# genome/breakdancer

Hardware: AMD Instinct MI355X
Metric: read-pairs/s, records resident in HBM -> scored SV table (SURVEY 8d timing i); end to end from BAM: config.timings.bam_to_table (vs_baseline is taken there) (higher is better)
Workload: dtype int32

## Files before the change

breakdancer_amd/csrc/bdx_api.hip:

```cpp
#include <hip/hip_runtime.h>

#include <algorithm>
#include <atomic>
#include <functional>
#include <memory>
#include <chrono>
#include <cmath>
#include <cstdio>
#include <cstddef>
#include <cstring>
#include <string>
#include <thread>
#include <unordered_map>
#include <utility>
#include <vector>

#include "../../include/bdx.h"
#include "bdx_buf.h"
#include "bdx_dev.h"
#include "bdx_k3.h"
#include "bdx_shard.h"
#include "bdx_scan.h"
#include "bdx_walk.h"
#include "bdx_bam_dev.h"

using namespace bdx;

namespace {

struct KdScratch {
    DevBuf bits, longbits, cnt;
    DevBuf work, wrun, starts, pre, cbase, table, multi;
    void release_long() { work.release(); wrun.release(); starts.release(); pre.release(); cbase.release(); table.release(); multi.release(); }
};

struct StageBufs {
    DevBuf b_c_tid, b_c_pos, b_c_isize, b_c_meta, b_c_key, b_c_check, b_c_idx, b_c_nn, b_c_pk;
    DevBuf b_cand, b_pre_q, b_pre_rev, b_pre_nonctx, b_c_first, b_c_maxq, b_c_rid, b_region_of, b_lb;
    DevBuf b_bcnt, b_boff, b_bcur, b_e_key, b_e_idx, b_partner, b_t_key, b_t_idx, b_pair_lo;
    DevBuf b_groups;
    DevBuf b_r_rec, b_r_pk, b_out_deg, b_parts, b_rs, b_slot, b_members, b_own, b_lib_stage, b_cn_stage, b_t_lambda, b_t_k, b_ws6;
    DevBuf b_sv_src, b_dlists, b_ltail, b_ins, b_member_ids;
    DevBuf b_sv_out, b_lib_index_out, b_lib_pairs_out, b_cn_key_out, b_cn_value_out, b_ltail_out, b_sv_key;
    PinBuf h_regs, h_pk, h_groups, h_counts0, h_counts2, h_sv_out, h_lib_index, h_lib_pairs, h_cn_key, h_cn_value, h_ltail_dev;
};

constexpr int kNumStages = 12;
enum StageMs { kMsClassify, kMsCompact, kMsCut, kMsJoinAssemble, kMsGroupsWait, kMsHostWalk, kMsFinish, kMsRun, kMsTableWait, kMsMerge, kMsScores };
enum ReadyWord { kPass1Ready, kGroupsReady, kTableReady, kRegionsReady };
constexpr int kK1MaxGrid = 8192;
constexpr uint32_t kK1EventPeriod = 4;

}

struct bdx_ctx {
    int device = 0;
    Stream stream;
    Stream copy_stream;
    bdx_opts opts{};
    std::vector<bdx_lib> libs;
    int nlibs = 0, nbams = 0, ntids = 0, nkeys = 0, w0 = 0;
    std::string err;

    ReadsSoA d{};
    size_t n = 0, cap = 0;
    bool adopted = false;
    DevBuf b_tid, b_pos, b_mtid, b_mpos, b_isize, b_flag, b_qlen, b_mapq, b_lib, b_bam, b_key, b_check;
    bool groups_in_hbm = false;
    bool use_check = false;

    DevBuf b_libs, b_cls, b_tile_tot, b_tile_pre, b_tile_mono, b_blk_cnt, b_cnt, b_p1, b_fold, b_stash, b_chunk_tot, b_counts;
    DevBuf b_lib_mean, b_kdens;
    PinBuf h_p1, h_cnt, h_counts, h_terms;
    PinBuf h_hs_rec, h_hs_aux, h_hs_lists, h_printed;
    StageBufs sb;
    PinBuf h_flags;
    PinBuf h_count;
    uint32_t seq = 0;
    int dbg_no_stash = 0, dbg_max_chunks = 0, dbg_ins_plain = 0, dbg_gather_walk = 0, dbg_regions_copy = 0, dbg_asm_plain = 0, dbg_depth_plain = 0;
    uint32_t lb_seq = 0;
    float k1_ms_last = 0;
    bool k1_timed = false;
    bool stage_timing = false;
    bool poll = true;
    bool materialized = true;
    bool rows_packed = false;
    uint32_t n_sv_total = 0, n_groups_total = 0, n_terms_total = 0, n_cn_total = 0;
    Event ev_groups, ev_regions;
    int big_walk_mode = -1;
    int64_t last_big_groups = -1;
    FinalizeParams fp_deferred{};
    bool finalize2_deferred = false;
    bool bucketed_join = false;
    bool host_walk_only = false;
    K6Arrays k6{};
    const GroupRec* k6_in_groups = nullptr;
    const uint32_t* k6_in_goff = nullptr;
    bool force_direct_join = false;
    uint32_t k6_cap = 0;
    const RegionRec* k6_r_rec = nullptr;
    const uint32_t* k6_r_pk = nullptr;
    uint8_t* k6_taint = nullptr;
    bool table_in_hbm = false;

    bool ran = false;
    Pass1 p1{};
    StageCounts counts{};
    std::vector<uint32_t> cnt;
    std::vector<uint32_t> cnt_local;
    uint32_t g_covered = 0;
    int32_t g_window = 0;
    uint32_t ntiles = 0, tstride = 0;
    Compact cp{};
    K3Arrays k3{};
    K4Arrays k4{};
    std::vector<double> log_tail;
    bool collect_support = false;
    std::vector<uint32_t> ov_cnt;
    uint32_t ov_covered = 0;
    bool replayed = false;
    bool use_stash = false;
    std::atomic<int> sizing{0};
    std::string sizing_err;
    std::vector<uint32_t> sup_off;
    std::vector<uint64_t> sup_idx;
    std::vector<uint8_t> sup_flag;
    std::vector<float> seqcov, lib_density, key_density;
    std::vector<HostRegion> regions;
    std::vector<uint32_t> r_pk;
    const HostRegion* reg = nullptr;
    size_t nreg = 0;
    const uint32_t* rpk = nullptr;
    std::vector<GroupPart> parts;
    WalkResult walk;
    std::unique_ptr<WalkScratch, void (*)(WalkScratch*)> walk_scratch{nullptr, walk_scratch_free};
    uint32_t n_printed = 0;
    uint32_t n_sv_host = 0;
    int speculate = 2;
    int spec_test = 0;
    uint32_t last_na = 0;
    size_t last_n = 0;
    uint32_t count_chunks = 0;
    uint32_t na_alloc = 0;
    bool region_of_fused = false;
    uint32_t join_table_clean = 0;
    float stage_ms[kNumStages] = {0};
    Event ev[8];

    Event ev_copy;
    bool copy_pending = false;
    bool k1_live = false;
    uint32_t k1_done = 0, k1_cap_tiles = 0;
    struct Stage {
        PinBuf buf;
        size_t cap = 0;
        Event done;
        bool busy = false;
    };
    Stage ring[4];
    int ring_next = 0, ring_cur = -1;
    struct KeySeg { uint64_t begin; const uint64_t* host; const uint16_t* host_qlen; const uint64_t* host_check; };
    std::vector<KeySeg> key_segs;
    DevBuf b_seg;

    size_t cls_n = (size_t)-1;
    DevBuf b_qtab;
    DevBuf b_qin, b_qout;
    bool mark_dup = false;
    bool dup_done = false;
    uint64_t dup_marked = 0, dup_groups = 0;
    KdScratch kd;
};

namespace {

// ... 452 lines not shown

int kd_run(bdx_ctx* c, KdParams p, KdScratch& k, uint16_t* flag, uint8_t* mask, hipStream_t s, uint64_t* marked, uint64_t* groups) {
    if (!p.n) return BDX_OK;
    const size_t nwords = (p.n + 63) / 64;
    HIPCHK(c, k.bits.ensure(nwords * 8));
    HIPCHK(c, k.longbits.ensure(nwords * 8));
    HIPCHK(c, k.cnt.ensure(sizeof(KdCounts)));
    p.bits = k.bits.as<uint64_t>(); p.longbits = k.longbits.as<uint64_t>(); p.cnt = k.cnt.as<KdCounts>();
    HIPCHK(c, hipMemsetAsync(p.cnt, 0, sizeof(KdCounts), s));
    launch_kd_scan(p, s);
    HIPCHK(c, hipGetLastError());
    KdCounts h{};
    HIPCHK(c, hipMemcpyAsync(&h, p.cnt, sizeof(h), hipMemcpyDeviceToHost, s));
    HIPCHK(c, hipStreamSynchronize(s));
    if (h.nwork) {
        if (h.nwork > (1u << 30)) return fail(c, BDX_ELIMIT, "more than 2^30 duplicate candidates in runs too long for direct comparison");
        uint64_t slots = 1024;
        while (slots < 2 * (uint64_t)h.nwork) slots <<= 1;
        HIPCHK(c, k.work.ensure((size_t)h.nwork * 4));
        HIPCHK(c, k.wrun.ensure((size_t)h.nwork * 4));
        HIPCHK(c, k.starts.ensure(nwords * 8));
        HIPCHK(c, k.pre.ensure(nwords * 4));
        HIPCHK(c, k.cbase.ensure((size_t)kd_chunks(p.n) * 4));
        HIPCHK(c, k.table.ensure(slots * 4));
        HIPCHK(c, k.multi.ensure(slots * 4));
        p.work = k.work.as<uint32_t>(); p.wrun = k.wrun.as<uint32_t>(); p.starts = k.starts.as<uint64_t>();
        p.pre = k.pre.as<uint32_t>(); p.cbase = k.cbase.as<uint32_t>();
        p.table = k.table.as<uint32_t>(); p.multi = k.multi.as<uint32_t>(); p.tmask = slots - 1;
        launch_kd_long(p, h.nwork, s);
        HIPCHK(c, hipGetLastError());
    }
    launch_kd_apply(p, flag, mask, s);
    HIPCHK(c, hipGetLastError());
    if (h.nwork) {
        HIPCHK(c, hipMemcpyAsync(&h, p.cnt, sizeof(h), hipMemcpyDeviceToHost, s));
        HIPCHK(c, hipStreamSynchronize(s));
        if (h.nlist != h.nwork) return fail(c, BDX_EINTERNAL, "duplicate marking: the work list does not hold the candidates that were counted");
        k.release_long();
    }
    *marked += h.marked; *groups += h.groups;
    return BDX_OK;
}

int mark_duplicates(bdx_ctx* c) {
    if (c->dup_done) return BDX_OK;
    c->dup_marked = 0; c->dup_groups = 0;
    hipStream_t s = c->stream;
    if (c->adopted && (const void*)c->d.flag != c->b_flag.p) {
        HIPCHK(c, c->b_flag.ensure(c->n * 2));
        HIPCHK(c, hipMemcpyAsync(c->b_flag.p, c->d.flag, c->n * 2, hipMemcpyDeviceToDevice, s));
        c->d.flag = c->b_flag.as<uint16_t>();
    }
    KdParams p{};
    p.tid = c->d.tid; p.pos = c->d.pos; p.mtid = c->d.mtid; p.mpos = c->d.mpos; p.flag = c->d.flag;
    p.lib = c->nlibs > 1 ? c->d.lib : nullptr;
    p.key = c->d.key; p.n = c->n;
    size_t ns = 0;
    BDX_TRY(upload_key_segs(c, &ns));
    if (ns) {
        p.nseg = (int)ns;
        p.seg_begin = c->b_seg.as<uint64_t>();
        p.seg_ptr = (const uint64_t* const*)(c->b_seg.as<uint64_t>() + ns + 1);
    }
    BDX_TRY(kd_run(c, p, c->kd, (uint16_t*)c->d.flag, nullptr, s, &c->dup_marked, &c->dup_groups));
    c->dup_done = true;
    return BDX_OK;
}

int pass1_prepare(bdx_ctx* c, uint32_t tiles_cap) {
    HIPCHK(c, hipSetDevice(c->device));
    hipStream_t s = c->stream;
    const int nlibs = c->nlibs, nbams = c->nbams, nkeys = c->nkeys;
    const int ncols = 2 + nkeys, ncnt = nlibs * kNumFlags + nlibs + nbams;
    const uint32_t tstride = (uint32_t)round_up(std::max<uint32_t>(tiles_cap, 16), 16);
    c->tstride = tstride;
    c->k1_cap_tiles = tiles_cap;
    c->k1_done = 0;
    HIPCHK(c, c->b_cls.ensure(std::max<size_t>((size_t)tiles_cap * kTile, 16)));
    c->use_stash = !c->dbg_no_stash && nkeys <= kStashKeys;
    if (c->use_stash) HIPCHK(c, c->b_stash.ensure(std::max<size_t>((size_t)tiles_cap * kStashCap * sizeof(StashRec), 64)));
    HIPCHK(c, c->b_tile_tot.ensure((size_t)ncols * tstride * 4));
    HIPCHK(c, c->b_tile_pre.ensure((size_t)ncols * tstride * 4));
    HIPCHK(c, c->b_tile_mono.ensure((size_t)nbams * tstride * sizeof(MonoRec)));
    HIPCHK(c, c->b_blk_cnt.ensure((size_t)kCntCopies * ncnt * 4));
    HIPCHK(c, c->b_cnt.ensure((size_t)ncnt * 4));
    HIPCHK(c, c->b_p1.ensure(sizeof(Pass1)));
    HIPCHK(c, c->h_p1.ensure(sizeof(Pass1)));
    HIPCHK(c, c->h_cnt.ensure((size_t)ncnt * 4));
    HIPCHK(c, c->h_counts.ensure(sizeof(StageCounts)));
    HIPCHK(c, c->b_counts.ensure(sizeof(StageCounts)));
    HIPCHK(c, c->h_count.ensure((size_t)kMaxChunks * 8));
    const size_t w_tot = (size_t)ncols * tstride, w_mono = (size_t)nbams * tstride * sizeof(MonoRec) / 4;
    if (w_tot > 0xFFFFFFFFull || w_mono > 0xFFFFFFFFull) {
        HIPCHK(c, hipMemsetAsync(c->b_tile_tot.p, 0, w_tot * 4, s));
        HIPCHK(c, hipMemsetAsync(c->b_tile_mono.p, 0xFF, w_mono * 4, s));
    }
    InitList il{};
    int k = 0;
    auto add = [&](void* p, size_t words, uint32_t value) { il.ptr[k] = (uint32_t*)p; il.words[k] = (uint32_t)words; il.value[k] = value; ++k; };
    if (w_tot <= 0xFFFFFFFFull && w_mono <= 0xFFFFFFFFull) { add(c->b_tile_tot.p, w_tot, 0u); add(c->b_tile_mono.p, w_mono, 0xFFFFFFFFu); }
    add(c->b_blk_cnt.p, (size_t)kCntCopies * ncnt, 0u);
    add(c->b_p1.p, sizeof(Pass1) / 4, 0u);
    add(c->b_counts.p, sizeof(StageCounts) / 4, 0u);
    il.n = k;
    launch_init(il, s);
    return BDX_OK;
}

int pass1_classify(bdx_ctx* c, uint32_t upto, bool timed) {
    hipStream_t s = c->stream;
    if (upto <= c->k1_done) return BDX_OK;
    K1Params k1{};
    k1.r = c->d; k1.n = c->n; k1.ntiles = upto; k1.tstride = c->tstride; k1.tile0 = c->k1_done;
    k1.nlibs = c->nlibs; k1.nbams = c->nbams; k1.nkeys = c->nkeys;
    k1.max_sd = c->opts.max_sd; k1.opt_t = c->opts.transchr_rearrange; k1.opt_l = c->opts.illumina_long_insert;
    k1.libs = c->b_libs.as<DevLib>(); k1.cls = c->b_cls.as<uint8_t>(); k1.tile_tot = c->b_tile_tot.as<uint32_t>();
    k1.tile_mono = c->b_tile_mono.as<MonoRec>();
    k1.blk_cnt = c->b_blk_cnt.as<uint32_t>();
    k1.stash = c->use_stash ? c->b_stash.as<StashRec>() : nullptr;
    const uint32_t span = upto - c->k1_done;
    const int grid1 = (int)std::min<uint32_t>((span + kWaves - 1) / kWaves, (uint32_t)kK1MaxGrid);
    launch_k1(k1, grid1, k1_lds_bytes(c->nlibs, c->nbams, c->nkeys), s, timed ? c->ev[0] : nullptr, timed ? c->ev[1] : nullptr);
    c->k1_done = upto;
    return BDX_OK;
}

struct Pass1Launch {
    uint32_t na_cap = 0;
    bool defer_second = false;
    bool post_count = false;
};
int pass1_finalize(bdx_ctx* c, const Pass1Launch& opt) {
    const int nlibs = c->nlibs, nbams = c->nbams, nkeys = c->nkeys;
    const int ncols = 2 + nkeys, ncnt = nlibs * kNumFlags + nlibs + nbams;
    const uint32_t ntiles = c->ntiles;
    FinalizeParams fp{};
    fp.ntiles = ntiles; fp.tstride = c->tstride; fp.nblk = 0;
    fp.nfold = std::max<uint32_t>(1, std::min<uint32_t>(64, (ntiles + 1023) / 1024));
    HIPCHK(c, c->b_fold.ensure((size_t)nbams * fp.nfold * sizeof(MonoRec)));
    fp.fold_part = c->b_fold.as<MonoRec>();
    fp.nlibs = nlibs; fp.nbams = nbams; fp.nkeys = nkeys; fp.ncols = ncols; fp.ncnt = ncnt; fp.w0 = c->w0;
    fp.tile_tot = c->b_tile_tot.as<uint32_t>(); fp.tile_pre = c->b_tile_pre.as<uint32_t>(); fp.tile_mono = c->b_tile_mono.as<MonoRec>();
    {
        const uint32_t nsuper = (ntiles + kK2TilesPerWave - 1) / kK2TilesPerWave;
        const uint32_t round = 4096;
        const uint32_t rounds = std::max<uint32_t>(1, (nsuper + round - 1) / round);
        const uint32_t max_chunks = c->dbg_max_chunks > 0 ? (uint32_t)std::min(c->dbg_max_chunks, (int)kMaxChunks) : (uint32_t)kMaxChunks;
        fp.chunk_super = round * ((rounds + max_chunks - 1) / max_chunks);
        fp.nchunk = std::max<uint32_t>(1, (nsuper + fp.chunk_super - 1) / fp.chunk_super);
        HIPCHK(c, c->b_chunk_tot.ensure((size_t)ncols * kMaxChunks * 8));
        fp.chunk_tot = c->b_chunk_tot.as<uint32_t>();
        fp.chunk_base = fp.chunk_tot + (size_t)ncols * kMaxChunks;
    }
    fp.blk_cnt = c->b_blk_cnt.as<uint32_t>(); fp.cnt = c->b_cnt.as<uint32_t>(); fp.p1 = c->b_p1.as<Pass1>();
    HIPCHK(c, c->b_kdens.ensure(64 * 4));
    fp.libs = c->b_libs.as<DevLib>(); fp.cn_lib = c->opts.cn_lib; fp.key_density = c->b_kdens.as<float>();
    fp.cnt_host = c->h_cnt.as<uint32_t>(); fp.p1_host = c->h_p1.as<Pass1>();
    memset(c->h_p1.p, 0, sizeof(Pass1));
    HIPCHK(c, c->h_flags.ensure(64));
    ++c->seq;
    fp.flag_host = c->h_flags.as<uint32_t>(); fp.flag_value = c->seq;
    fp.na_cap = opt.na_cap;
    fp.count_host = opt.post_count && c->poll ? c->h_count.as<uint64_t>() : nullptr; fp.count_stamp = c->seq;
    c->count_chunks = fp.count_host ? fp.nchunk : 0;
    c->fp_deferred = fp;
    c->finalize2_deferred = opt.defer_second;
    launch_finalize(fp, c->stream, !opt.defer_second);
    return BDX_OK;
}

int do_pass1(bdx_ctx* c, const Pass1Launch& opt) {
    HIPCHK(c, hipSetDevice(c->device));
    hipStream_t s = c->stream;
    if (c->n >= ((size_t)1 << 32)) return fail(c, BDX_ELIMIT, "more than 2^32 - 1 reads in one context (read indices and the prefix counters are 32-bit)");
    const uint32_t ntiles = (uint32_t)((c->n + kTile - 1) / kTile);
    c->ntiles = ntiles;
    c->ran = false; c->replayed = false;
    c->cls_n = (size_t)-1;
    c->na_alloc = 0;
    c->regions.clear(); c->r_pk.clear(); c->parts.clear();
    c->reg = nullptr; c->nreg = 0; c->rpk = nullptr;
    c->walk.clear();
    if (!c->walk_scratch) c->walk_scratch.reset(walk_scratch_new());
    c->n_printed = 0;
    memset(&c->counts, 0, sizeof(c->counts));
    for (float& m : c->stage_ms) m = 0;

    if (c->copy_pending) {
        HIPCHK(c, hipStreamWaitEvent(s, c->ev_copy, 0));
        c->copy_pending = false;
    }
    if (!(c->k1_live && c->k1_cap_tiles >= ntiles)) {
        BDX_TRY(pass1_prepare(c, ntiles));
    }
    c->k1_live = false;
    if (c->mark_dup && c->k1_done == 0) {
        BDX_TRY(mark_duplicates(c));
    }
    const bool time_k1 = (c->stage_timing || c->seq % kK1EventPeriod == 0) && c->k1_done == 0 && ntiles > 0;
    BDX_TRY(pass1_classify(c, ntiles, time_k1));
    BDX_TRY(pass1_finalize(c, opt));
    c->k1_timed = time_k1;
    return BDX_OK;
}

int wait_pass1(bdx_ctx* c) {
    const int ncnt = c->nlibs * kNumFlags + c->nlibs + c->nbams;
    BDX_TRY(await_ready(c, kPass1Ready, nullptr, "the pass-1 record did not arrive: its kernel was not launched", true));
    c->p1 = *c->h_p1.as<Pass1>();
    c->cnt_local.assign(c->h_cnt.as<uint32_t>(), c->h_cnt.as<uint32_t>() + ncnt);
    if (c->k1_timed) {
        float ms = 0;
        if (hipEventElapsedTime(&ms, c->ev[0], c->ev[1]) == hipSuccess) c->k1_ms_last = ms;
    }
    c->stage_ms[kMsClassify] = c->k1_ms_last;
    if (c->p1.n_anom > kMaxAnomalous) return fail(c, BDX_ELIMIT, "more than 2^31 anomalous reads in one context");
    if (!c->na_alloc && c->p1.n_anom) c->na_alloc = (uint32_t)std::min<uint64_t>(with_headroom(c->p1.n_anom), kMaxAnomalous);
    c->cls_n = c->n;
    return BDX_OK;
}

int32_t window_from(const bdx_ctx* c, const uint32_t* cnt, uint32_t covered) {
    int W = c->w0;
    for (int i = 0; i < c->nlibs; ++i) {
        const int nd = (int)(cnt[i * kNumFlags + F_LARGE] + cnt[i * kNumFlags + F_SMALL]);
        const int tmp = nd > 0 ? (int)((float)covered / (float)nd) : 50;
        W = std::min(W, tmp);
    }
    return W;
}

int set_pass1(bdx_ctx* c, const uint32_t* cnt, uint32_t covered, int32_t window, bool upload) {
    const int nlibs = c->nlibs, nkeys = c->nkeys;
    const int ncnt = nlibs * kNumFlags + nlibs + c->nbams;
    c->cnt.assign(cnt, cnt + ncnt);
    c->g_covered = covered;
    c->g_window = window;
    const uint32_t* lib_cnt = c->cnt.data() + nlibs * kNumFlags;
    const uint32_t* bam_cnt = lib_cnt + nlibs;
    c->seqcov.assign(nlibs, 0.f);
    c->lib_density.assign(nlibs, 0.f);
    c->key_density.assign(nkeys, 0.000001f);
    for (int i = 0; i < nlibs; ++i) {
        float covg = 0;
        if (lib_cnt[i] != 0 && covered != 0) covg = float(lib_cnt[i]) * c->libs[i].readlens / covered;
        c->seqcov[i] = covg;
        float dens = 0.000001f;
        if (c->opts.cn_lib) {
            if (lib_cnt[i] != 0) dens = float(lib_cnt[i]) / covered;
        } else {
// ... 86 lines not shown
    k.p2 = 1;
    while (k.p2 < k.sv) k.p2 <<= 1;
    k.nsort = std::min<size_t>(k.sv, kK6RankSortMax);
    return k;
}

int size_k6(StageBufs& b, const StageDims& d, hipStream_t s, std::string* err) {
    const size_t cap = d.k6_regions();
    if (!cap) return BDX_OK;
    const K6Caps k = k6_caps(d);
    SZCHK(size_out_deg(b, cap));
    SZCHK(b.b_parts.ensure(cap * sizeof(PartRec)));
    SZCHK(b.b_rs.ensure(cap * sizeof(RegSum)));
    SZCHK(b.b_members.ensure(cap * kK6MaxMembers * sizeof(MemberInfo)));
    SZCHK(b.b_own.ensure(cap * 7 * 4 + 64 * 4 * 4));
    if (d.walks_big()) SZCHK(b.b_member_ids.ensure(cap * kK6BigMembers * 4));
    SZCHK(b.b_slot.ensure(cap * sizeof(SvOut)));
    SZCHK(b.b_lib_stage.ensure(cap * k.lib_stride * sizeof(LibStage)));
    SZCHK(b.b_cn_stage.ensure(cap * (size_t)d.nkeys * sizeof(CnStage) + 16));
    SZCHK(b.b_t_lambda.ensure((size_t)k.term * 8)); SZCHK(b.b_t_k.ensure((size_t)k.term * 4));
    if (d.table_in_hbm) {
        SZCHK(b.b_sv_out.ensure((size_t)k.sv * sizeof(SvOut))); SZCHK(b.b_sv_key.ensure((size_t)k.sv * 8));
        SZCHK(b.b_lib_index_out.ensure((size_t)k.term * 4)); SZCHK(b.b_lib_pairs_out.ensure((size_t)k.term * 4));
        SZCHK(b.b_cn_key_out.ensure((size_t)k.cn * 4 + 16)); SZCHK(b.b_cn_value_out.ensure((size_t)k.cn * 4 + 16));
        SZCHK(b.b_ltail_out.ensure((size_t)k.term * 8));
    } else {
        SZCHK(b.h_sv_out.ensure((size_t)k.sv * sizeof(SvOut)));
        SZCHK(b.h_lib_index.ensure((size_t)k.term * 4)); SZCHK(b.h_lib_pairs.ensure((size_t)k.term * 4));
        SZCHK(b.h_cn_key.ensure((size_t)k.cn * 4 + 16)); SZCHK(b.h_cn_value.ensure((size_t)k.cn * 4 + 16));
        SZCHK(b.h_ltail_dev.ensure((size_t)k.term * 8));
    }
    SZCHK(b.h_counts2.ensure(sizeof(StageCounts)));
    SZCHK(b.b_sv_src.ensure((size_t)k.sv * 16)); SZCHK(b.b_ltail.ensure((size_t)k.term * 8));
    SZCHK(b.b_dlists.ensure((size_t)k.term * 4 + (size_t)k.cn * 8 + 64));
    SZCHK(b.b_ins.ensure(k.p2 * 12 + (size_t)k.sv * 8 + ((size_t)k.sv + 1) * 16 + k.nsort * 12 + k.nsort * 4 * kK6RankSlices + 64));
    SZCHK(size_zero_once(b.b_ws6, 4 * (scan_grid((uint32_t)cap, 1) + 1) * 8, s));
    return BDX_OK;
}

int do_compact(bdx_ctx* c) {
    HIPCHK(c, hipSetDevice(c->device));
    hipStream_t s = c->stream;
    const int nkeys = c->nkeys;
    const uint32_t na = c->na_alloc;
    if (c->stage_timing) HIPCHK(c, hipEventRecord(c->ev[2], s));
    Compact& cp = c->cp;
    cp = Compact{};
    c->k3 = K3Arrays{};
    if (na) {
        const StageDims dm = stage_dims(c, na);
        BDX_TRY(size_compact(c->sb, dm, &c->err));
        const StageBufs& b = c->sb;
        cp.tid = b.b_c_tid.as<int32_t>(); cp.pos = b.b_c_pos.as<int32_t>(); cp.isize = b.b_c_isize.as<int32_t>();
        cp.meta = b.b_c_meta.as<uint32_t>(); cp.key = b.b_c_key.as<uint64_t>(); cp.nn = b.b_c_nn.as<uint32_t>();
        cp.idx = b.b_c_idx.as<uint32_t>();
        cp.check = c->use_check ? b.b_c_check.as<uint64_t>() : nullptr;
        cp.pk = b.b_c_pk.as<uint32_t>(); cp.cap = na;
        K2Params k2{};
        k2.r = c->d; k2.n = c->n; k2.ntiles = c->ntiles; k2.tstride = c->tstride; k2.nkeys = nkeys; k2.nlibs = c->nlibs; k2.libs = c->b_libs.as<DevLib>();
        k2.cls = c->b_cls.as<uint8_t>(); k2.tile_pre = c->b_tile_pre.as<uint32_t>(); k2.c = cp;
        k2.tile_tot = c->b_tile_tot.as<uint32_t>(); k2.stash = c->use_stash ? c->b_stash.as<StashRec>() : nullptr;
        k2.chunk_tot = c->fp_deferred.chunk_tot; k2.chunk_base = c->fp_deferred.chunk_base; k2.chunk_super = c->fp_deferred.chunk_super;
        k2.fill_ptr[0] = b.b_c_maxq.as<uint32_t>(); k2.fill_words[0] = na; k2.fill_value[0] = 0u;
        c->join_table_clean = 0;
        if (dm.k2_clears_join) {
            const uint32_t slots = dm.join_slots;
            k2.fill_ptr[1] = b.b_t_key.as<uint32_t>(); k2.fill_words[1] = 2 * slots; k2.fill_value[1] = 0xFFFFFFFFu;
            k2.fill_ptr[2] = b.b_partner.as<uint32_t>(); k2.fill_words[2] = na; k2.fill_value[2] = 0xFFFFFFFFu;
            k2.fill_ptr[3] = b.b_pair_lo.as<uint32_t>(); k2.fill_words[3] = na; k2.fill_value[3] = 0xFFFFFFFFu;
            c->join_table_clean = slots;
        }
        {
            size_t ns = 0;
            BDX_TRY(upload_key_segs(c, &ns));
            if (ns) {
                k2.nseg = (int)ns;
                k2.seg_begin = c->b_seg.as<uint64_t>();
                k2.seg_ptr = (const uint64_t* const*)(c->b_seg.as<uint64_t>() + ns + 1);
                k2.seg_qlen = (const uint16_t* const*)(c->b_seg.as<uint64_t>() + 2 * ns + 1);
                k2.seg_check = (const uint64_t* const*)(c->b_seg.as<uint64_t>() + 3 * ns + 1);
            }
        }
        launch_k2(k2, k2_lds_bytes(nkeys), s, c->finalize2_deferred ? &c->fp_deferred : nullptr);
        c->finalize2_deferred = false;
    }
    if (c->finalize2_deferred) {
        launch_finalize2_only(c->fp_deferred, s);
        c->finalize2_deferred = false;
    }
    if (c->stage_timing) HIPCHK(c, hipEventRecord(c->ev[3], s));
    return BDX_OK;
}

void own_borrowed_regions(bdx_ctx* c) {
    if (!c->reg || (const void*)c->reg != c->sb.h_regs.p) return;
    const HostRegion* r = c->reg;
    const uint32_t* pk = c->rpk;
    const size_t n = c->nreg;
    std::vector<HostRegion> keep(r, r + n);
    std::vector<uint32_t> keep_pk;
    if (pk) keep_pk.assign(pk, pk + n * 2 * (size_t)c->nkeys);
    c->regions.swap(keep); c->r_pk.swap(keep_pk);
    c->reg = c->regions.data(); c->rpk = c->r_pk.data();
}

int do_cut(bdx_ctx* c, const uint32_t* tid_tail, RegionDst dst) {
    HIPCHK(c, hipSetDevice(c->device));
    hipStream_t s = c->stream;
    const uint32_t na = c->na_alloc;
    if (na) {
        StageDims dm = stage_dims(c, na);
        dm.regions = dst;
        BDX_TRY(size_cut(c->sb, dm, s, &c->err));
        const StageBufs& b = c->sb;
        K3Arrays& k3 = c->k3;
        const bool for_k6 = dst == RegionDst::HostAndHbm;
        k3.cap = na;
        k3.cand = b.b_cand.as<int32_t>(); k3.pre_q = b.b_pre_q.as<uint32_t>(); k3.pre_rev = b.b_pre_rev.as<uint32_t>();
        k3.pre_nonctx = b.b_pre_nonctx.as<uint32_t>(); k3.c_first = b.b_c_first.as<uint32_t>();
        k3.c_maxq = b.b_c_maxq.as<int32_t>(); k3.c_rid = b.b_c_rid.as<int32_t>(); k3.region_of = b.b_region_of.as<int32_t>();
        k3.r_rec = for_k6 ? b.h_regs.as<RegionRec>() : b.b_r_rec.as<RegionRec>();
        k3.r_pk = for_k6 ? b.h_pk.as<uint32_t>() : b.b_r_pk.as<uint32_t>();
        if (for_k6) {
            k3.r_rec_dev = b.b_r_rec.as<RegionRec>(); k3.r_pk_dev = b.b_r_pk.as<uint32_t>(); k3.out_deg = b.b_out_deg.as<uint32_t>();
            k3.host_copy_later = joins_direct(c, na) ? 1 : 0;
            memset(b.h_counts0.p, 0, sizeof(StageCounts));
            k3.counts_host = b.h_counts0.as<StageCounts>();
        } else {
            k3.r_rec_dev = nullptr; k3.r_pk_dev = nullptr; k3.host_copy_later = 0;
        }
        k3.lb_state = b.b_lb.as<unsigned long long>();
        HIPCHK(c, next_lb_stamp(c, &k3.lb_stamp));
        k3.counts = c->b_counts.as<StageCounts>();
        c->region_of_fused = for_k6 && joins_direct(c, na);
        launch_k3(k3, c->cp, c->b_p1.as<Pass1>(), na, c->opts.min_len, c->opts.seq_coverage_lim, c->nkeys, tid_tail, !c->region_of_fused, s);
        if (for_k6 && !k3.host_copy_later) {
            BDX_TRY(signal_ready(c, kRegionsReady, c->ev_regions));
        }
    }
    if (c->stage_timing) HIPCHK(c, hipEventRecord(c->ev[4], s));
    return BDX_OK;
}

int do_join_local(bdx_ctx* c, uint32_t n, const Entries& en, const uint32_t* n_ptr) {
    hipStream_t s = c->stream;
    K4Arrays& k4 = c->k4;
    k4 = K4Arrays{};
    if (!n) return BDX_OK;
    const bool direct = joins_direct(c, n);
    StageDims dm = stage_dims(c, c->na_alloc);
    dm.join_n = n;
    dm.join_own = en.n_local ? std::min<uint32_t>(n, std::max<uint32_t>(c->na_alloc, 1u)) : n;
    dm.join_slots = !direct ? 0u : (c->join_table_clean && (uint64_t)n * 2 <= c->join_table_clean) ? c->join_table_clean : direct_join_slots(n);
    dm.join_pair_lo = en.want_pair_lo != 0;
    BDX_TRY(size_join(c->sb, dm, &c->err));
    StageBufs& b = c->sb;
    k4.g_cap = dm.join_groups();
    k4.g_rec = c->groups_in_hbm ? b.b_groups.as<GroupRec>() : b.h_groups.as<GroupRec>();
    k4.partner = b.b_partner.as<int32_t>();
    if (direct) {
        const uint32_t slots = dm.join_slots;
        const size_t n_own = dm.join_own;
        const bool want_lo = en.c_rid || en.want_pair_lo;
        if (c->join_table_clean != slots) {
            HIPCHK(c, hipMemsetAsync(b.b_t_key.p, 0xFF, (size_t)slots * 8, s));
            HIPCHK(c, hipMemsetAsync(b.b_partner.p, 0xFF, n_own * 4, s));
            if (en.want_pair_lo) HIPCHK(c, hipMemsetAsync(b.b_pair_lo.p, 0xFF, n_own * 4, s));
        }
        k4.pair_lo = ((c->join_table_clean == slots && want_lo) || en.want_pair_lo) ? b.b_pair_lo.as<int32_t>() : nullptr;
        c->join_table_clean = 0;
// ... 1057 lines not shown
```

breakdancer_amd/csrc/bdx_dev.h:

```cpp
#pragma once
#include <hip/hip_runtime.h>
#include <stdint.h>

namespace bdx {

constexpr int kTile = 256;
constexpr int kBlock = 256;
constexpr int kWaves = kBlock / 64;
constexpr int kNumFlags = 11;
constexpr int kK2TilesPerWave = 4;
constexpr int kCntCopies = 64;
constexpr int kMaxChunks = 64;
constexpr int kStashCap = 16;
constexpr int kStashKeys = 2;

struct StashRec {
    int32_t tid, pos, isize;
    uint32_t meta;
    uint32_t where;
    uint32_t proper;
    uint32_t pad[2];
};
static_assert(sizeof(StashRec) == 32, "two 16-byte stores");

enum : int { F_NA = 0, F_FF = 1, F_LARGE = 2, F_SMALL = 3, F_RF = 4, F_RR = 5, F_NORMAL_FR = 6, F_NORMAL_RF = 7,
             F_CTX = 8, F_MATE_UNMAPPED = 9, F_UNMAPPED = 10 };

struct DevLib {
    float upper, lower;
    int32_t min_mapq;
    int32_t key;
};

struct ReadsSoA {
    const int32_t *tid, *pos, *mtid, *mpos, *isize;
    const uint16_t *flag, *qlen;
    const uint8_t *mapq, *lib, *bam;
    const uint64_t* key;
    const uint64_t* check;
};

struct MonoRec {
    int32_t ft, fp, lt, lp;
    long long sum;
};

constexpr int kColAnom = 0, kColNormal = 1, kColKey0 = 2;

struct K1Params {
    ReadsSoA r;
    uint64_t n;
    uint32_t ntiles, tstride;
    uint32_t tile0;
    int nlibs, nbams, nkeys;
    int max_sd, opt_t, opt_l;
    const DevLib* libs;
    uint8_t* cls;
    uint32_t* tile_tot;
    MonoRec* tile_mono;
    uint32_t* blk_cnt;
    StashRec* stash;
};

struct Pass1 {
    uint32_t covered_ref_len;
    int32_t window;
    uint32_t n_anom;
    uint32_t n_normal;
    uint32_t key_tot[60];
    unsigned long long ref_len[256];
};

struct FinalizeParams {
    uint32_t ntiles, tstride, nblk;
    uint32_t nfold;
    MonoRec* fold_part;
    int nlibs, nbams, nkeys, ncols, ncnt;
    int w0;
    const uint32_t* tile_tot;
    uint32_t* tile_pre;
    uint32_t* chunk_tot;
    uint32_t* chunk_base;
    uint32_t chunk_super, nchunk;
    const MonoRec* tile_mono;
    const uint32_t* blk_cnt;
    uint32_t* cnt;
    Pass1* p1;
    uint32_t* cnt_host;
    Pass1* p1_host;
    const DevLib* libs;
    int cn_lib;
    float* key_density;
    uint32_t* flag_host;
    uint32_t flag_value;
    uint64_t* count_host;
    uint32_t count_stamp;
    uint32_t na_cap;
};

struct InitList {
    uint32_t* ptr[6];
    uint32_t words[6];
    uint32_t value[6];
    int n;
};
void launch_init(const InitList& l, hipStream_t s);

struct Compact {
    int32_t* tid;
    int32_t* pos;
    int32_t* isize;
    uint32_t* meta;
    uint64_t* key;
    uint64_t* check;
    uint32_t* idx;
    uint32_t* nn;
    uint32_t* pk;
    uint32_t cap;
};

struct K2Params {
    ReadsSoA r;
    uint64_t n;
    uint32_t ntiles, tstride;
    int nkeys, nlibs;
    const DevLib* libs;
    const uint8_t* cls;
    const uint32_t* tile_pre;
    const uint32_t* chunk_tot;
    const uint32_t* chunk_base;
    uint32_t chunk_super;
    const uint32_t* tile_tot;
    const StashRec* stash;
    Compact c;
    uint32_t* fill_ptr[4];
    uint32_t fill_words[4];
    uint32_t fill_value[4];
    int nseg;
    const uint64_t* seg_begin;
    const uint64_t* const* seg_ptr;
    const uint16_t* const* seg_qlen;
    const uint64_t* const* seg_check;
};

__device__ __forceinline__ uint32_t meta_pack(int flag, int rev, int lib, int qlen) {
    return (uint32_t)flag | ((uint32_t)rev << 4) | ((uint32_t)lib << 8) | ((uint32_t)qlen << 16);
}
__host__ __device__ __forceinline__ int meta_flag(uint32_t m) { return m & 15; }
__host__ __device__ __forceinline__ int meta_rev(uint32_t m) { return (m >> 4) & 1; }
__host__ __device__ __forceinline__ int meta_lib(uint32_t m) { return (m >> 8) & 255; }
__host__ __device__ __forceinline__ int meta_qlen(uint32_t m) { return m >> 16; }

__device__ __forceinline__ int lane_id() { return threadIdx.x & 63; }
__device__ __forceinline__ int wave_id() { return threadIdx.x >> 6; }
__device__ __forceinline__ uint64_t ballot64(bool p) { return __builtin_amdgcn_ballot_w64(p); }
__device__ __forceinline__ int popc64(uint64_t m) { return __popcll(m); }

__device__ __forceinline__ uint32_t wave_incl_scan(uint32_t v) {
    const int l = lane_id();
#pragma unroll
    for (int o = 1; o < 64; o <<= 1) {
        uint32_t t = __shfl_up(v, o);
        if (l >= o) v += t;
    }
    return v;
}

struct StoreView {
    const int32_t *tid, *pos, *mtid, *mpos, *isize;
    const uint16_t* flag;
    const uint8_t* cls;
    uint64_t n;
};

struct K8Params {
    StoreView st;
    const uint8_t* key;
    const int32_t *q_tid, *q_a, *q_b;
    uint32_t nq;
// ... 111 lines not shown
```

breakdancer_amd/csrc/bdx_finalize.h:

```cpp
#pragma once
#include <cstddef>

#include "bdx_dev.h"

namespace bdx {

__device__ __forceinline__ MonoRec mono_combine(const MonoRec& a, const MonoRec& b) {
    if (a.ft == -1) return b;
    if (b.ft == -1) return a;
    MonoRec r;
    r.ft = a.ft; r.fp = a.fp; r.lt = b.lt; r.lp = b.lp;
    r.sum = a.sum + b.sum + (a.lt == b.ft ? (long long)b.fp - (long long)a.lp : 0ll);
    return r;
}
__device__ __forceinline__ MonoRec mono_shfl_down(const MonoRec& a, int o) {
    MonoRec r;
    r.ft = __shfl_down(a.ft, o); r.fp = __shfl_down(a.fp, o); r.lt = __shfl_down(a.lt, o); r.lp = __shfl_down(a.lp, o);
    r.sum = __shfl_down(a.sum, o);
    return r;
}

__device__ __forceinline__ void finalize2_body(const FinalizeParams& p) {
    __shared__ uint32_t s_acc[255 * 12 + 256];
    __shared__ unsigned long long s_ref[256];
    __shared__ uint32_t s_head[2];
    __shared__ uint32_t s_col[64];
    const int t = threadIdx.x, lane = t & 63, w = t >> 6;
    for (int i = t; i < p.ncnt; i += 256) s_acc[i] = 0;
    __syncthreads();
    for (int idx = t; idx < kCntCopies * p.ncnt; idx += 256) {
        const uint32_t v = p.blk_cnt[idx];
        if (v) atomicAdd(&s_acc[idx % p.ncnt], v);
    }
    __syncthreads();
    for (int i = t; i < p.ncnt; i += 256) {
        const uint32_t v = s_acc[i];
        p.cnt[i] = v;
        if (p.cnt_host) p.cnt_host[i] = v;
    }
    for (int c0 = 0; c0 < p.ncols; c0 += 4) {
        const int c = c0 + w;
        uint32_t v = (c < p.ncols && (uint32_t)lane < p.nchunk) ? p.chunk_tot[(size_t)c * kMaxChunks + lane] : 0u;
        {
            uint32_t inc = v;
#pragma unroll
            for (int o = 1; o < 64; o <<= 1) {
                const uint32_t u = __shfl_up(inc, o);
                if (lane >= o) inc += u;
            }
            if (c < p.ncols) p.chunk_base[(size_t)c * kMaxChunks + lane] = inc - v;
        }
#pragma unroll
        for (int o = 32; o > 0; o >>= 1) v += __shfl_xor(v, o);
        if (lane == 0 && c < p.ncols) {
            s_col[c] = v;
            if (c == kColAnom) p.p1->n_anom = v;
            else if (c == kColNormal) p.p1->n_normal = v;
            else p.p1->key_tot[c - kColKey0] = v;
        }
    }
    for (int b0 = 0; b0 < p.nbams; b0 += 4) {
        const int b = b0 + w;
        MonoRec acc;
        acc.ft = -1; acc.fp = 0; acc.lt = 0; acc.lp = 0; acc.sum = 0;
        if (b < p.nbams && (uint32_t)lane < p.nfold) acc = p.fold_part[(size_t)b * p.nfold + lane];
#pragma unroll
        for (int o = 1; o < 64; o <<= 1) {
            const MonoRec other = mono_shfl_down(acc, o);
            if (lane + o < 64 && ((lane & (2 * o - 1)) == 0)) acc = mono_combine(acc, other);
        }
        if (lane == 0 && b < p.nbams) {
            const unsigned long long r = acc.ft == -1 ? 0ull : (unsigned long long)acc.sum;
            s_ref[b] = r;
            p.p1->ref_len[b] = r;
        }
    }
    __syncthreads();
    if (t == 0) {
        uint32_t covered = 0;
        for (int b = 0; b < p.nbams; ++b)
            if ((unsigned long long)covered < s_ref[b]) covered = (uint32_t)s_ref[b];
        p.p1->covered_ref_len = covered;
        int W = p.w0;
        for (int i = 0; i < p.nlibs; ++i) {
            const int nd = (int)(s_acc[i * kNumFlags + F_LARGE] + s_acc[i * kNumFlags + F_SMALL]);
            const int tmp = nd > 0 ? (int)__fdiv_rn((float)covered, (float)nd) : 50;
            W = min(W, tmp);
        }
        p.p1->window = W;
        s_head[0] = covered; s_head[1] = (uint32_t)W;
        if (p.key_density) {
            const uint32_t* lib_cnt = s_acc + p.nlibs * kNumFlags;
            const uint32_t* bam_cnt = lib_cnt + p.nlibs;
            for (int k = 0; k < p.nkeys; ++k) p.key_density[k] = 0.000001f;
            for (int i = 0; i < p.nlibs; ++i) {
                const int key = p.libs[i].key;
                float dens = 0.000001f;
                if (p.cn_lib) {
                    if (lib_cnt[i] != 0) dens = __fdiv_rn((float)lib_cnt[i], (float)covered);
                } else {
                    dens = __fdiv_rn((float)bam_cnt[key], (float)covered);
                }
                p.key_density[key] = dens;
            }
        }
    }
    if (p.p1_host) {
        __syncthreads();
        uint32_t* dst = (uint32_t*)p.p1_host;
        static_assert(offsetof(Pass1, covered_ref_len) == 0 && offsetof(Pass1, window) == 4 && offsetof(Pass1, n_anom) == 8 &&
                          offsetof(Pass1, n_normal) == 12 && offsetof(Pass1, key_tot) == 16 && offsetof(Pass1, ref_len) % 8 == 0, "Pass1 mirror");
        static_assert(kColAnom == 0 && kColNormal == 1 && kColKey0 == 2, "the record's words 2.. are the column totals in column order");
        constexpr int kRefWord = (int)(offsetof(Pass1, ref_len) / 4);
        const int words = kRefWord + 2 * p.nbams;
        for (int i = t; i < words; i += 256) {
            uint32_t v;
// ... 19 lines not shown
```

breakdancer_amd/csrc/k1_classify.hip:

```cpp
#include <cstddef>

#include <hip/hip_ext.h>

#include "bdx_dev.h"
#include "bdx_finalize.h"

#include <limits.h>

#ifdef BDX_KPROF
#include "bdx_scan.h"
#else
#define KPROF(row, col) do {} while (0)
#endif

namespace bdx {

constexpr int kMixedLibs = 8;

typedef int v4i __attribute__((ext_vector_type(4)));
typedef unsigned short v4us __attribute__((ext_vector_type(4)));
typedef unsigned char v4uc __attribute__((ext_vector_type(4)));
__device__ __forceinline__ int4 ldnt(const int32_t* p) { const v4i v = __builtin_nontemporal_load((const v4i*)p); return make_int4(v.x, v.y, v.z, v.w); }
__device__ __forceinline__ ushort4 ldnt(const uint16_t* p) { const v4us v = __builtin_nontemporal_load((const v4us*)p); return make_ushort4(v.x, v.y, v.z, v.w); }
__device__ __forceinline__ uchar4 ldnt(const uint8_t* p) { const v4uc v = __builtin_nontemporal_load((const v4uc*)p); return make_uchar4(v.x, v.y, v.z, v.w); }
// ... 524 lines not shown
                    pending &= ~mine;
                    const uint64_t M = ballot64(mine != 0);
                    const int fl = __ffsll((long long)M) - 1, ll = 63 - __clzll((long long)M);
                    const int fs = mine ? __ffs(mine) - 1 : 0, ls = mine ? 31 - __clz(mine) : 0;
                    const int first = __shfl(pos[fs], fl), last = __shfl(pos[ls], ll);
                    if (lane_m == (int)v) { present = true; my_first = first; my_last = last; }
                }
                if (present) {
                    MonoRec m;
                    m.ft = tw; m.fp = my_first; m.lt = tw; m.lp = my_last; m.sum = (long long)my_last - (long long)my_first;
                    p.tile_mono[(size_t)lane_m * p.tstride + tile] = m;
                }
            } else {
                if (lane_m == 0)
                    for (int b = 0; b < nbams_m; ++b) my_mono[b].ft = -1;
                for (int L = 0; L < 64; ++L) {
#pragma unroll
                    for (int r = 0; r < 4; ++r) {
                        const int nv = __shfl(nvalid, L);
                        if (r >= nv) continue;
                        const int rt = __shfl(tid[r], L), rp = __shfl(pos[r], L);
                        const unsigned rb = __shfl(bam[r], L);
                        if (lane_m == 0) {
                            MonoRec m = my_mono[rb];
                            if (m.ft == -1) { m.ft = rt; m.fp = rp; m.sum = 0; }
                            else if (m.lt == rt) m.sum += (long long)rp - (long long)m.lp;
                            m.lt = rt; m.lp = rp;
                            my_mono[rb] = m;
                        }
                    }
                }
                if (lane_m == 0)
                    for (int b = 0; b < nbams_m; ++b)
                        if (my_mono[b].ft != -1) p.tile_mono[(size_t)b * p.tstride + tile] = my_mono[b];
            }
            }
        }
    }
    __syncthreads();
    uint32_t* out = p.blk_cnt + (size_t)(blockIdx.x & (kCntCopies - 1)) * ncnt;
    for (int i = t; i < ncnt; i += kBlock) {
        const uint32_t v = s_cnt[i];
        if (v) atomicAdd(&out[i], v);
    }
}

void launch_k1(const K1Params& p, int grid, size_t lds, hipStream_t s, hipEvent_t start, hipEvent_t stop) {
    auto kernel = p.opt_l ? k1_classify_kernel<true> : k1_classify_kernel<false>;
    if (start && stop) hipExtLaunchKernelGGL(kernel, dim3(grid), dim3(kBlock), (uint32_t)lds, s, start, stop, 0u, p);
    else hipLaunchKernelGGL(kernel, dim3(grid), dim3(kBlock), lds, s, p);
}

constexpr int kFinBlock = 1024;

__global__ __launch_bounds__(kFinBlock) void finalize_kernel(const FinalizeParams p) {
    __shared__ uint32_t s_carry;
    __shared__ MonoRec s_mono[kFinBlock / 64];
    const int t = threadIdx.x, lane = t & 63, w = t >> 6;
    KPROF(blockIdx.x * 16 + w, 0);

    const uint32_t nscan = (uint32_t)p.ncols * p.nchunk;
    if (blockIdx.x < nscan) {
        const int c = (int)(blockIdx.x / p.nchunk);
        const uint32_t g = blockIdx.x % p.nchunk;
        const uint32_t tile_lo = g * p.chunk_super * kK2TilesPerWave;
        const uint32_t tile_hi = min(p.ntiles, (g + 1) * p.chunk_super * kK2TilesPerWave);
        const uint32_t* in = p.tile_tot + (size_t)c * p.tstride;
        uint32_t* out = p.tile_pre + (size_t)c * p.tstride;
        if (t == 0) s_carry = 0;
        __syncthreads();
        constexpr int kQ = 4;
        static_assert(kK2TilesPerWave == 4 && kFinBlock == 1024, "one 16-byte load per super tile");
        __shared__ uint32_t s_wt[kQ * (kFinBlock / 64)];
        __shared__ uint32_t s_round;
        const uint32_t row_hi = min(p.tstride, (g + 1) * p.chunk_super * kK2TilesPerWave);
        volatile uint64_t* const count_word = (c == kColAnom && t == 0 && p.count_host) ? p.count_host + g : nullptr;
        if (count_word && tile_lo >= tile_hi) *count_word = (uint64_t)p.count_stamp << 32;
        for (uint32_t base = tile_lo; base < tile_hi; base += kFinBlock * kQ * 4) {
            uint32_t sum[kQ], inc[kQ];
#pragma unroll
            for (int q = 0; q < kQ; ++q) {
                const uint32_t i = base + ((uint32_t)q * kFinBlock + t) * 4;
                uint4 x = make_uint4(0, 0, 0, 0);
                if (i < row_hi) x = *(const uint4*)(in + i);
                sum[q] = x.x + x.y + x.z + x.w;
            }
            if (sum[0] != 0xFFFFFFFFu) KPROF(blockIdx.x * 16 + w, 1);
#pragma unroll
            for (int q = 0; q < kQ; ++q) inc[q] = wave_incl_scan(sum[q]);
            if (lane == 63) {
#pragma unroll
                for (int q = 0; q < kQ; ++q) s_wt[q * (kFinBlock / 64) + w] = inc[q];
            }
            __syncthreads();
            if (w == 0) {
                static_assert(kQ * (kFinBlock / 64) == 64, "one wave total per lane");
                const uint32_t v = s_wt[lane];
                const uint32_t li = wave_incl_scan(v);
                s_wt[lane] = li - v;
                if (lane == 63) s_round = li;
            }
            __syncthreads();
            if (count_word && tile_hi - base <= (uint32_t)(kFinBlock * kQ * 4)) *count_word = ((uint64_t)p.count_stamp << 32) | (uint32_t)(s_carry + s_round);
#pragma unroll
            for (int q = 0; q < kQ; ++q) {
                const uint32_t i = base + ((uint32_t)q * kFinBlock + t) * 4;
                if (i < row_hi) out[i / 4] = s_carry + s_wt[q * (kFinBlock / 64) + w] + inc[q] - sum[q];
            }
            __syncthreads();
            if (t == 0) s_carry += s_round;
            __syncthreads();
        }
        if (t == 0) p.chunk_tot[(size_t)c * kMaxChunks + g] = s_carry;
        KPROF(blockIdx.x * 16 + w, 2);
        return;
    }

    const uint32_t fb = blockIdx.x - nscan;
    const uint32_t chunk = (p.ntiles + p.nfold - 1) / p.nfold;
    const uint32_t c0 = fb * chunk, c1 = min(c0 + chunk, p.ntiles);
    const uint32_t per = (chunk + kFinBlock - 1) / kFinBlock;
    for (int b = 0; b < p.nbams; ++b) {
        const MonoRec* mo = p.tile_mono + (size_t)b * p.tstride;
        MonoRec acc;
        acc.ft = -1; acc.fp = 0; acc.lt = 0; acc.lp = 0; acc.sum = 0;
        const uint32_t t0 = min(c0 + (uint32_t)t * per, c1), t1 = min(t0 + per, c1);
        for (uint32_t i = t0; i < t1; i += 8) {
            MonoRec e[8];
#pragma unroll
            for (int q = 0; q < 8; ++q) {
                if (i + q < t1) e[q] = mo[i + q];
                else e[q].ft = -1;
            }
#pragma unroll
            for (int q = 0; q < 8; ++q) acc = mono_combine(acc, e[q]);
        }
        if (acc.ft != -12345) KPROF(blockIdx.x * 16 + w, 1);
#pragma unroll
        for (int o = 1; o < 64; o <<= 1) {
            const MonoRec other = mono_shfl_down(acc, o);
            if (lane + o < 64 && ((lane & (2 * o - 1)) == 0)) acc = mono_combine(acc, other);
        }
        if (lane == 0) s_mono[w] = acc;
        __syncthreads();
        if (t == 0) {
            MonoRec tot = s_mono[0];
            for (int k = 1; k < kFinBlock / 64; ++k) tot = mono_combine(tot, s_mono[k]);
            p.fold_part[(size_t)b * p.nfold + fb] = tot;
        }
        __syncthreads();
    }
    KPROF(blockIdx.x * 16 + w, 2);
}

__global__ __launch_bounds__(256) void finalize2_kernel(const FinalizeParams p) { finalize2_body(p); }

__global__ __launch_bounds__(256) void k0_init_kernel(const InitList l) {
    for (int f = 0; f < l.n; ++f)
        for (uint32_t i = blockIdx.x * 256 + threadIdx.x; i < l.words[f]; i += gridDim.x * 256) l.ptr[f][i] = l.value[f];
}

void launch_init(const InitList& l, hipStream_t s) {
    uint32_t mx = 0;
    for (int f = 0; f < l.n; ++f) mx = l.words[f] > mx ? l.words[f] : mx;
    if (!mx) return;
    const uint32_t g = (mx + 1023) / 1024;
    hipLaunchKernelGGL(k0_init_kernel, dim3(g < 1024u ? g : 1024u), dim3(256), 0, s, l);
}
// ... 22 lines not shown
```

Baseline: 29.28 billion.

## Drop per-pass zero-init of tile totals; self-clear counters inside finalize

The pass1 init launch no longer zeroes the tile_tot array. Instead, the finalize scan masks reads past tile_hi so stale padding cannot leak into the sums. Per-block counters are cleared by the finalize kernel as it consumes them, tracked by a dirty flag, and the StageCounts buffer is zeroed inside finalize. The mono init is skipped for single-BAM runs, which cuts init memory traffic at the cost of relying on k1 to overwrite every tile_tot entry up to ntiles.

Result: faster. 29.62 billion (median of 6 runs) (+1.1%).

```diff
diff --git a/breakdancer_amd/csrc/bdx_api.hip b/breakdancer_amd/csrc/bdx_api.hip
--- a/breakdancer_amd/csrc/bdx_api.hip
+++ b/breakdancer_amd/csrc/bdx_api.hip
@@ -91,6 +91,7 @@
     int64_t last_big_groups = -1;
     FinalizeParams fp_deferred{};
     bool finalize2_deferred = false;
+    bool blk_cnt_dirty = false;
     bool bucketed_join = false;
     bool host_walk_only = false;
     K6Arrays k6{};
@@ -709,7 +710,11 @@
     HIPCHK(c, c->b_tile_tot.ensure((size_t)ncols * tstride * 4));
     HIPCHK(c, c->b_tile_pre.ensure((size_t)ncols * tstride * 4));
     HIPCHK(c, c->b_tile_mono.ensure((size_t)nbams * tstride * sizeof(MonoRec)));
-    HIPCHK(c, c->b_blk_cnt.ensure((size_t)kCntCopies * ncnt * 4));
+    if (c->b_blk_cnt.bytes < (size_t)kCntCopies * ncnt * 4) {
+        HIPCHK(c, c->b_blk_cnt.ensure((size_t)kCntCopies * ncnt * 4));
+        HIPCHK(c, hipMemsetAsync(c->b_blk_cnt.p, 0, c->b_blk_cnt.bytes, s));
+        c->blk_cnt_dirty = false;
+    }
     HIPCHK(c, c->b_cnt.ensure((size_t)ncnt * 4));
     HIPCHK(c, c->b_p1.ensure(sizeof(Pass1)));
     HIPCHK(c, c->h_p1.ensure(sizeof(Pass1)));
@@ -717,18 +722,16 @@
     HIPCHK(c, c->h_counts.ensure(sizeof(StageCounts)));
     HIPCHK(c, c->b_counts.ensure(sizeof(StageCounts)));
     HIPCHK(c, c->h_count.ensure((size_t)kMaxChunks * 8));
-    const size_t w_tot = (size_t)ncols * tstride, w_mono = (size_t)nbams * tstride * sizeof(MonoRec) / 4;
-    if (w_tot > 0xFFFFFFFFull || w_mono > 0xFFFFFFFFull) {
-        HIPCHK(c, hipMemsetAsync(c->b_tile_tot.p, 0, w_tot * 4, s));
-        HIPCHK(c, hipMemsetAsync(c->b_tile_mono.p, 0xFF, w_mono * 4, s));
-    }
+    const size_t w_mono = (size_t)nbams * tstride * sizeof(MonoRec) / 4;
     InitList il{};
     int k = 0;
     auto add = [&](void* p, size_t words, uint32_t value) { il.ptr[k] = (uint32_t*)p; il.words[k] = (uint32_t)words; il.value[k] = value; ++k; };
-    if (w_tot <= 0xFFFFFFFFull && w_mono <= 0xFFFFFFFFull) { add(c->b_tile_tot.p, w_tot, 0u); add(c->b_tile_mono.p, w_mono, 0xFFFFFFFFu); }
-    add(c->b_blk_cnt.p, (size_t)kCntCopies * ncnt, 0u);
-    add(c->b_p1.p, sizeof(Pass1) / 4, 0u);
-    add(c->b_counts.p, sizeof(StageCounts) / 4, 0u);
+    if (nbams > 1) {
+        if (w_mono > 0xFFFFFFFFull) HIPCHK(c, hipMemsetAsync(c->b_tile_mono.p, 0xFF, w_mono * 4, s));
+        else add(c->b_tile_mono.p, w_mono, 0xFFFFFFFFu);
+    }
+    if (c->blk_cnt_dirty) add(c->b_blk_cnt.p, (size_t)kCntCopies * ncnt, 0u);
+    c->blk_cnt_dirty = false;
     il.n = k;
     launch_init(il, s);
     return BDX_OK;
@@ -747,6 +750,7 @@
     k1.stash = c->use_stash ? c->b_stash.as<StashRec>() : nullptr;
     const uint32_t span = upto - c->k1_done;
     const int grid1 = (int)std::min<uint32_t>((span + kWaves - 1) / kWaves, (uint32_t)kK1MaxGrid);
+    c->blk_cnt_dirty = true;
     launch_k1(k1, grid1, k1_lds_bytes(c->nlibs, c->nbams, c->nkeys), s, timed ? c->ev[0] : nullptr, timed ? c->ev[1] : nullptr);
     c->k1_done = upto;
     return BDX_OK;
@@ -787,12 +791,14 @@
     HIPCHK(c, c->h_flags.ensure(64));
     ++c->seq;
     fp.flag_host = c->h_flags.as<uint32_t>(); fp.flag_value = c->seq;
+    fp.zero_ptr = c->b_counts.as<uint32_t>(); fp.zero_words = sizeof(StageCounts) / 4;
     fp.na_cap = opt.na_cap;
     fp.count_host = opt.post_count && c->poll ? c->h_count.as<uint64_t>() : nullptr; fp.count_stamp = c->seq;
     c->count_chunks = fp.count_host ? fp.nchunk : 0;
     c->fp_deferred = fp;
     c->finalize2_deferred = opt.defer_second;
     launch_finalize(fp, c->stream, !opt.defer_second);
+    if (!opt.defer_second) c->blk_cnt_dirty = false;
     return BDX_OK;
 }
 
@@ -1045,10 +1051,12 @@
             }
         }
         launch_k2(k2, k2_lds_bytes(nkeys), s, c->finalize2_deferred ? &c->fp_deferred : nullptr);
+        if (c->finalize2_deferred) c->blk_cnt_dirty = false;
         c->finalize2_deferred = false;
     }
     if (c->finalize2_deferred) {
         launch_finalize2_only(c->fp_deferred, s);
+        c->blk_cnt_dirty = false;
         c->finalize2_deferred = false;
     }
     if (c->stage_timing) HIPCHK(c, hipEventRecord(c->ev[3], s));
diff --git a/breakdancer_amd/csrc/bdx_dev.h b/breakdancer_amd/csrc/bdx_dev.h
--- a/breakdancer_amd/csrc/bdx_dev.h
+++ b/breakdancer_amd/csrc/bdx_dev.h
@@ -83,7 +83,7 @@
     uint32_t* chunk_base;
     uint32_t chunk_super, nchunk;
     const MonoRec* tile_mono;
-    const uint32_t* blk_cnt;
+    uint32_t* blk_cnt;
     uint32_t* cnt;
     Pass1* p1;
     uint32_t* cnt_host;
@@ -95,6 +95,8 @@
     uint32_t flag_value;
     uint64_t* count_host;
     uint32_t count_stamp;
+    uint32_t* zero_ptr;
+    uint32_t zero_words;
     uint32_t na_cap;
 };
 
diff --git a/breakdancer_amd/csrc/bdx_finalize.h b/breakdancer_amd/csrc/bdx_finalize.h
--- a/breakdancer_amd/csrc/bdx_finalize.h
+++ b/breakdancer_amd/csrc/bdx_finalize.h
@@ -30,8 +30,9 @@
     __syncthreads();
     for (int idx = t; idx < kCntCopies * p.ncnt; idx += 256) {
         const uint32_t v = p.blk_cnt[idx];
-        if (v) atomicAdd(&s_acc[idx % p.ncnt], v);
+        if (v) { atomicAdd(&s_acc[idx % p.ncnt], v); p.blk_cnt[idx] = 0u; }
     }
+    for (uint32_t i = t; i < p.zero_words; i += 256) p.zero_ptr[i] = 0u;
     __syncthreads();
     for (int i = t; i < p.ncnt; i += 256) {
         const uint32_t v = s_acc[i];
diff --git a/breakdancer_amd/csrc/k1_classify.hip b/breakdancer_amd/csrc/k1_classify.hip
--- a/breakdancer_amd/csrc/k1_classify.hip
+++ b/breakdancer_amd/csrc/k1_classify.hip
@@ -630,8 +630,8 @@
             for (int q = 0; q < kQ; ++q) {
                 const uint32_t i = base + ((uint32_t)q * kFinBlock + t) * 4;
                 uint4 x = make_uint4(0, 0, 0, 0);
-                if (i < row_hi) x = *(const uint4*)(in + i);
-                sum[q] = x.x + x.y + x.z + x.w;
+                if (i < tile_hi) x = *(const uint4*)(in + i);
+                sum[q] = x.x + (i + 1 < tile_hi ? x.y : 0u) + (i + 2 < tile_hi ? x.z : 0u) + (i + 3 < tile_hi ? x.w : 0u);
             }
             if (sum[0] != 0xFFFFFFFFu) KPROF(blockIdx.x * 16 + w, 1);
 #pragma unroll
```
